# hrpan/tetris_mcts

Hardware: NVIDIA H100
Metric: mcts_sims_per_sec (higher is better)
Workload: dtype f32

## Files before the change

tetris_mcts_b200/_lib.py:

```python
import ctypes as C
import os

import numpy as np

HERE = os.path.dirname(os.path.abspath(__file__))
LIB_PATH = os.environ.get("B200_TETRIS_LIB") or os.path.join(HERE, "libb200_tetris_mcts.so")

REC_WORDS = 20
KEY_WORDS = 12
N_ACTIONS = 7
N_WEIGHTS = 478342

MODE_LP, MODE_SINGLE, MODE_VANILLA, MODE_DIST = 0, 1, 2, 3
EVAL_SYNTHETIC, EVAL_NET, EVAL_NET_TC = 0, 1, 2
ERR_NAMES = {1: "BAD_ARG", 2: "CUDA", 3: "ARENA_FULL", 4: "TRACE_FULL", 5: "NO_WEIGHTS"}


class B200Error(RuntimeError):
    def __init__(self, code, msg):
        super().__init__("b200 error %d (%s): %s" % (code, ERR_NAMES.get(code, "?"), msg))
        self.code = code


class Config(C.Structure):
# ... 13 lines not shown
    if _lib is None:
        if not os.path.exists(LIB_PATH):
            raise ImportError("%s is missing: run `python -m tetris_mcts_b200.build` (nvcc, sm_90a). "
                              "tetris_mcts_b200 has no CPU fallback." % LIB_PATH)
        L = C.CDLL(LIB_PATH)
        L.b200_last_error.restype = C.c_char_p
        L.b200_engine_create.argtypes = [C.POINTER(Config), C.POINTER(P)]
        L.b200_engine_destroy.argtypes = [P]
        L.b200_engine_set_stream.argtypes = [P, P]
        L.b200_engine_get_stream.argtypes = [P, C.POINTER(P)]
        L.b200_load_weights.argtypes = [P, P]
        L.b200_set_games.argtypes = [P, P]
        L.b200_get_games.argtypes = [P, P]
        L.b200_update_root.argtypes = [P, C.c_int]
        L.b200_run_sims.argtypes = [P, C.c_int]
        L.b200_get_stats.argtypes = [P, P, P]
        L.b200_env_step.argtypes = [P, P]
        L.b200_play_move.argtypes = [P, C.c_int, C.c_int, P, P]
        L.b200_status.argtypes = [P, P]
        L.b200_finished_games.argtypes = [P, P, C.c_int, P]
        L.b200_remove_nodes.argtypes = [P, C.c_int]
        L.b200_set_gc_headroom.argtypes = [P, C.c_int]
        L.b200_set_deep_lane.argtypes = [P, C.c_int]
        L.b200_set_path_cache.argtypes = [P, C.c_int]
        L.b200_counters.argtypes = [P, P]
        L.b200_sync.argtypes = [P]
        L.b200_set_timing.argtypes = [P, C.c_int]
        L.b200_timer_start.argtypes = [P]
        L.b200_timer_stop.argtypes = [P, P]
        L.b200_phase_ms.argtypes = [P, P, P]
        L.b200_export_game.argtypes = [P, C.c_int] + [P] * 13
        L.b200_valuenet_forward.argtypes = [P, P, C.c_int, P, P]
        L.b200_debug_act3.argtypes = [P, P, C.c_int, P]
        L.b200_tetris_step.argtypes = [P, P, C.c_int]
        L.b200_tetris_new.argtypes = [P, C.c_int, C.c_int, C.c_int, C.c_int, P, C.c_int]
        L.b200_tetris_state.argtypes = [P, P, C.c_int]
        L.b200_select_trace_obs.argtypes = [C.c_int] + [P] * 6 + [C.c_int, C.c_int, P, P, C.c_int, P]
        L.b200_backup_trace_obs.argtypes = [P, C.c_int] + [P] * 5 + [C.c_int, C.c_double, C.c_double, C.c_double]
        L.b200_backup_trace_obs_LP.argtypes = ([P, C.c_int] + [P] * 6 + [C.c_int, P, P, C.c_int, P, P, C.c_double,
                                               C.c_int, C.c_int])
        L.b200_get_unique_child_obs.argtypes = [C.c_int, P, P, P, C.c_int, P, P, P]
        L.b200_get_all_childs.argtypes = [C.c_int, P, C.c_int, P]
        L.b200_collect_samples_dev.argtypes = [P, C.c_int, P, C.c_int, P]
        L.b200_replay_enable.argtypes = [P, C.c_int, C.c_int]
        L.b200_replay_drain_dev.argtypes = [P, P, C.c_int, P]
        L.b200_replay_policy.argtypes = [P, C.c_int, C.c_int, C.c_int]
        L.b200_replay_policy_step.argtypes = [P, C.c_int64, P, P]
        L.b200_replay_policy_trained.argtypes = [P, C.c_int64]
        L.b200_replay_peek_dev.argtypes = [P, P, C.c_int]
        L.b200_replay_append.argtypes = [P, P, C.c_int]
        L.b200_load_dist_weights.argtypes = [P, P, C.c_int]
        L.b200_distnet_forward.argtypes = [P, P, C.c_int, C.c_int, P]
        L.b200_export_dist.argtypes = [P, C.c_int, P, P]
        L.b200_dist_shift_distribution.argtypes = [P, C.c_int, C.c_double, C.c_double, C.c_double, P]
        L.b200_dist_mean_variance.argtypes = [P, C.c_int, C.c_double, C.c_double, P, P]
        L.b200_dist_select_trace.argtypes = [C.c_int, P, P, C.c_int, C.c_int, P, P, C.c_int, P]
        L.b200_dist_backup_trace.argtypes = [P, C.c_int, P, P, C.c_int, C.c_int, C.c_double, P, C.c_double, C.c_double]
        _lib = L
    return _lib


def check(rc):
    if rc != 0:
        raise B200Error(rc, lib().b200_last_error().decode())


# ... 10 lines not shown
```

tetris_mcts_b200/csrc/capi.cu:

```cuda
#include <cuda_runtime.h>
#include <cmath>
#include <cstdio>
#include <cstdlib>
#include <cstring>
#include <string>
#include <vector>

#include "../../include/b200_tetris_mcts.h"
#include "kernels.cuh"
#include "valuenet_simt.cuh"
#include "dist_dev.cuh"
#include "distnet_simt.cuh"
#include "replay_policy.cuh"
#ifdef B200_WITH_TC
#include "valuenet_tc.cuh"
#include "distnet_tc.cuh"
#endif

using namespace b200;

static thread_local std::string g_err;
static int fail(int code, const std::string &msg) { g_err = msg; return code; }
#define CK(call)                                                                                      \
    do {                                                                                              \
// ... 18 lines not shown
    std::vector<void *> allocs;
    uint32_t *d_default_rec = nullptr;
    float *d_stats = nullptr; int32_t *d_action = nullptr;
    unsigned long long *d_game_stats = nullptr;
    bool have_weights = false;
    float *d_wraw = nullptr;
    NetWeights W{};
    float *d_act3 = nullptr; size_t act3_rows = 0;
    void *tc_state = nullptr; void *dn_tc_state = nullptr;
    bool have_dist_weights = false; float *d_dnw = nullptr; DistNetWeights DW{}; float *d_dn_act = nullptr; size_t dn_rows = 0;
    int n_sm = 132;
    bool timing = false;
    std::vector<cudaEvent_t> ev; size_t ev_used = 0;
    std::vector<int> ev_phase;
    float phase_ms[PH_N] = {0}; uint64_t phase_launches[PH_N] = {0};
    cudaEvent_t t0 = nullptr, t1 = nullptr;
    uint8_t *d_samples = nullptr; int sample_cap = 0; int32_t *d_sample_count = nullptr;
    ReplayPolicy rp; uint8_t *d_rp_tmp = nullptr, *d_rp_keep = nullptr; float *d_rp_vis = nullptr; int32_t *d_rp_kept = nullptr; int replay_alloc = 0;
    int gc_headroom = 0;
    int4 *d_pc = nullptr; int32_t *d_pc_var = nullptr, *d_pc_len = nullptr; uint4 *d_pc_sib = nullptr; int4 *d_pc_own = nullptr;
    int deep_cap = 0; cudaStream_t stream1 = nullptr; cudaEvent_t ev_fork = nullptr, ev_join = nullptr;
    int32_t *d_glist0 = nullptr, *d_glist1 = nullptr, *d_nlist = nullptr, *d_nreq_deep = nullptr, *d_gc_list_deep = nullptr; uint2 *d_req_deep = nullptr;
    int gc_pool_main = 0;
    cudaGraphExec_t step_exec = nullptr; bool step_graph_failed = false;
    uint64_t step_launches[PH_N] = {0};
};

static void drop_step_graph(b200_engine *e) {
    if (e->step_exec) { cudaStreamSynchronize(e->stream); cudaGraphExecDestroy(e->step_exec); e->step_exec = nullptr; }
    e->step_graph_failed = false;
}

constexpr int DEEP_GC_BLOCKS = 8;

static inline int backup_bitmap_words(const Arena &A) { return A.pc ? (A.M + 31) / 32 : 0; }
static inline size_t backup_smem(const Arena &A) { return (size_t)4 * backup_bitmap_words(A) * sizeof(unsigned); }

struct Scratch {
    std::vector<void *> bufs;
    ~Scratch() { for (void *q : bufs) cudaFree(q); }
    template <typename T> cudaError_t get(T **out, size_t bytes) {
        void *q = nullptr;
        cudaError_t err = cudaMalloc(&q, bytes ? bytes : 1);
        if (err == cudaSuccess) { bufs.push_back(q); *out = (T *)q; }
        return err;
    }
};

static void dfree(b200_engine *e, void *p) {
    if (!p) return;
    for (size_t i = 0; i < e->allocs.size(); ++i)
        if (e->allocs[i] == p) { e->allocs.erase(e->allocs.begin() + i); break; }
    cudaFree(p);
}

template <typename T>
static int dalloc(b200_engine *e, T **p, size_t n, bool zero = true) {
    void *q = nullptr;
    cudaError_t err = cudaMalloc(&q, n * sizeof(T));
    if (err != cudaSuccess) return fail(B200_ERR_CUDA, std::string("cudaMalloc ") + std::to_string(n * sizeof(T)) + " B: " + cudaGetErrorString(err));
    if (zero) cudaMemsetAsync(q, 0, n * sizeof(T), e->stream);
    e->allocs.push_back(q);
    *p = (T *)q;
    return 0;
}

// ... 67 lines not shown
    cudaDeviceProp prop;
    CK(cudaGetDeviceProperties(&prop, cfg->device));
    e->n_sm = prop.multiProcessorCount;
    Arena &A = e->A;
    memset(&A, 0, sizeof(A));
    A.G = cfg->n_games; A.M = cfg->max_nodes;
    int H = A.M + A.M / 2;
    if (H < 16) H = 16;
    A.H = H; A.trace_max = cfg->trace_max > 0 ? cfg->trace_max : 512;
    A.mode = cfg->mode; A.low = cfg->low; A.lp_end_from_obs = cfg->lp_end_from_obs; A.lp_var_gamma2 = cfg->lp_var_gamma2;
    A.stale_pop = cfg->stale_pop; A.eval_kind = cfg->eval_kind; A.overflow_reset = cfg->overflow_reset; A.gc_min_gain = cfg->overflow_reset ? cfg->max_nodes / 8 : 0; A.gamma = cfg->gamma; A.rollout_variance = cfg->rollout_variance;
    size_t GM = (size_t)A.G * A.M, G = (size_t)A.G;
    int rc = 0;
    rc |= dalloc(e, &A.row, GM * ROW_WORDS);
    rc |= dalloc(e, &A.stat, GM);
    rc |= dalloc(e, &A.rec, GM * REC_WORDS, false);
    rc |= dalloc(e, &A.key, GM * KEY_WORDS);
    rc |= dalloc(e, &A.ntab, G * H);
    rc |= dalloc(e, &A.otab, G * H);
    rc |= dalloc(e, &A.nfree, GM); rc |= dalloc(e, &A.ofree, GM);
    rc |= dalloc(e, &A.n_nfree, G); rc |= dalloc(e, &A.n_ofree, G);
    rc |= dalloc(e, &A.root, G); rc |= dalloc(e, &A.episode, G); rc |= dalloc(e, &A.status, G); rc |= dalloc(e, &A.srng, G);
    rc |= dalloc(e, &A.trace, G * A.trace_max); rc |= dalloc(e, &A.trace_len, G); rc |= dalloc(e, &A.leaf_kind, G);
    rc |= dalloc(e, &A.trace_meta, G * A.trace_max);
    {
        e->gc_pool_main = e->n_sm * 4 < A.G ? e->n_sm * 4 : A.G;
        const size_t pool = (size_t)(e->gc_pool_main + DEEP_GC_BLOCKS) * A.M;
        rc |= dalloc(e, &A.nmark, pool); rc |= dalloc(e, &A.omark, pool); rc |= dalloc(e, &A.gc_queue, pool * 2);
    }
    rc |= dalloc(e, &A.cur, G * REC_WORDS);
    rc |= dalloc(e, &A.req, G * 8); rc |= dalloc(e, &A.n_req, 4);
    rc |= dalloc(e, &A.gc_list, G); rc |= dalloc(e, &A.pending, G); rc |= dalloc(e, &A.resume_a, G);
    rc |= dalloc(e, &A.eval_out, G * 8); rc |= dalloc(e, &A.rollout_val, G);
    rc |= dalloc(e, &A.counters, 48);
    A.fin_cap = 4 * A.G;
    rc |= dalloc(e, &A.fin_log, (size_t)A.fin_cap * 4); rc |= dalloc(e, &A.fin_count, 1);
    if (cfg->mode == MODE_DIST) {
        A.dist_bins = cfg->dist_bins; A.dist_vmin = cfg->dist_vmin; A.dist_vmax = cfg->dist_vmax;
        rc |= dalloc(e, &A.nstat, GM * NSTAT_WORDS); rc |= dalloc(e, &A.ndist, GM * (size_t)A.dist_bins); rc |= dalloc(e, &A.dist_eval, G * (size_t)A.dist_bins);
    }
    rc |= dalloc(e, &e->d_default_rec, REC_WORDS);
    rc |= dalloc(e, &e->d_stats, G * 21); rc |= dalloc(e, &e->d_action, G);
    e->d_game_stats = A.counters + 8;
    float *zt = nullptr;
    rc |= dalloc(e, &zt, ZTABLE_N);
    if (rc) return B200_ERR_CUDA;
    {
        std::vector<float> h(ZTABLE_N);
        const double l2 = log(2.0), l22 = log(22.0), l41 = log(41.0);
        for (int n = 0; n < ZTABLE_N; ++n) {
            double t = (double)n, alpha = 1 - 1 / t;
            h[n] = (float)(10 * log(1 - log(-log(alpha) / l2) / l22) / l41);
        }
        CK(cudaMemcpyAsync(zt, h.data(), ZTABLE_N * sizeof(float), cudaMemcpyHostToDevice, e->stream));
        CK(cudaStreamSynchronize(e->stream));
        A.ztable = zt;
    }
    k_new_games<<<1, 1, 0, e->stream>>>(e->d_default_rec, 1, cfg->actions_per_drop, cfg->scoring, cfg->randomizer, nullptr, 0);
    k_init_arena<<<e->n_sm * 8, 256, 0, e->stream>>>(A, e->d_default_rec, cfg->seed);
    CK(cudaGetLastError());
    CK(cudaStreamSynchronize(e->stream));
    guard.e = nullptr;
    *out = e;
    return B200_OK;
}

extern "C" int b200_engine_destroy(b200_engine *e) {
// ... 73 lines not shown
    e->W.wfc1 = e->W.b1 + 96; e->W.bfc1 = e->W.wfc1 + (size_t)1792 * 256; e->W.wout = e->W.bfc1 + 256;
    e->W.bout = e->W.wout + 512; e->W.ub = e->W.bout + 2; e->W.lb = e->W.bout + 4;
    CK(cudaFuncSetAttribute(k_vn_conv, cudaFuncAttributeMaxDynamicSharedMemorySize, VN_SMEM_BYTES));
#ifdef B200_WITH_TC
    {
        int rc = tc_prepare(&e->tc_state, w, e->stream);
        if (rc) return fail(B200_ERR_CUDA, "tensor-core weight preparation failed");
    }
#endif
    e->have_weights = true;
    drop_step_graph(e);
    return B200_OK;
}

static int ensure_act3(b200_engine *e, size_t rows) {
    if (e->act3_rows >= rows) return 0;
    if (e->d_act3) { cudaStreamSynchronize(e->stream); dfree(e, e->d_act3); e->d_act3 = nullptr; e->act3_rows = 0; }
    if (dalloc(e, &e->d_act3, rows * 1792, false)) return B200_ERR_CUDA;
    e->act3_rows = rows;
    return 0;
}

static int launch_net(b200_engine *e, const uint2 *req, const int32_t *n_req, const uint32_t *keys, int M, float2 *eval_out,
                      size_t max_rows) {
    if (!e->have_weights) return fail(B200_ERR_NO_WEIGHTS, "b200_load_weights was not called");
#ifdef B200_WITH_TC
    if (e->cfg.eval_kind == B200_EVAL_NET_TC) {
        TcState *st = (TcState *)e->tc_state;
        const uint8_t *act3_before = st->d_act3;
        if (tc_ensure_act3(st, max_rows, e->stream)) return fail(B200_ERR_CUDA, "act3 (tensor-core layout) allocation failed");
        if (act3_before && st->d_act3 != act3_before) drop_step_graph(e);
        {
            PhaseTimer t(e, PH_CONV);
            k_tc_conv<<<e->n_sm, TCC_THREADS, TCC_SMEM, e->stream>>>(e->W, st->TW, req, n_req, nullptr, keys, M, st->d_act3, (int)st->tiles,
                                                                    e->timing ? e->A.counters + 16 : nullptr);
        }
        {
            PhaseTimer t(e, PH_FC);
            k_tc_fc<<<e->n_sm, TCF_THREADS, TCF_SMEM, e->stream>>>(e->W, st->TW, st->d_act3, (int)st->tiles, req, n_req, eval_out);
        }
        CK(cudaGetLastError());
        return B200_OK;
    }
#endif
    {
        const float *act3_before = e->d_act3;
        if (ensure_act3(e, max_rows)) return B200_ERR_CUDA;
        if (act3_before && e->d_act3 != act3_before) drop_step_graph(e);
    }
    {
        PhaseTimer t(e, PH_CONV);
        k_vn_conv<<<e->n_sm, VN_THREADS, VN_SMEM_BYTES, e->stream>>>(e->W, req, n_req, keys, M, e->d_act3);
    }
    {
        PhaseTimer t(e, PH_FC);
        k_vn_fc<<<e->n_sm * 2, FC_THREADS, 0, e->stream>>>(e->W, e->d_act3, req, n_req, eval_out);
    }
    CK(cudaGetLastError());
    return B200_OK;
}

__global__ void k_states_to_keys(const int8_t *states, int k, uint32_t *keys, uint2 *req);

extern "C" int b200_load_dist_weights(b200_engine *e, const float *w, int atoms) {
    if (!e || !w || atoms < 2 || atoms > 64) return fail(B200_ERR_BAD_ARG, "bad argument");
    CK(cudaSetDevice(e->cfg.device));
    if (e->A.mode == MODE_DIST && atoms != e->A.dist_bins) return fail(B200_ERR_BAD_ARG, "atoms must equal dist_bins");
    std::vector<float> h;
// ... 206 lines not shown
static int enqueue_step_lanes(b200_engine *e) {
    const Arena &A = e->A;
    const int G = A.G;
    if (!e->have_weights) return fail(B200_ERR_NO_WEIGHTS, "b200_load_weights was not called");
    TcState *st = (TcState *)e->tc_state;
    const uint8_t *act3_before = st->d_act3;
    if (tc_ensure_act3(st, (size_t)G * (A.mode == MODE_LP ? 7 : 1), e->stream)) return fail(B200_ERR_CUDA, "act3 (tensor-core layout) allocation failed");
    if (act3_before && st->d_act3 != act3_before) drop_step_graph(e);
    cudaStream_t s0 = e->stream, s1 = e->timing ? e->stream : e->stream1;
    Arena A0 = A, A1 = A;
    A0.glist = e->d_glist0; A0.n_list = e->d_nlist;
    A1.glist = e->d_glist1; A1.n_list = e->d_nlist + 1;
    A1.req = e->d_req_deep; A1.n_req = e->d_nreq_deep; A1.gc_list = e->d_gc_list_deep;
    A1.nmark += (size_t)e->gc_pool_main * A.M; A1.omark += (size_t)e->gc_pool_main * A.M; A1.gc_queue += (size_t)e->gc_pool_main * A.M * 2;
    A0.prof = e->timing ? A.counters + 32 : nullptr;
    CK(cudaMemsetAsync(A.n_req, 0, 4 * sizeof(int32_t), s0));
    CK(cudaMemsetAsync(e->d_nreq_deep, 0, 2 * sizeof(int32_t), s0));
    if (s1 != s0) { CK(cudaEventRecord(e->ev_fork, s0)); CK(cudaStreamWaitEvent(s1, e->ev_fork, 0)); }
    const int deep_groups = blocks_groups(e->deep_cap);
    {
        PhaseTimer t(e, PH_SELECT);
        k_select_expand<<<(G + SE_GAMES_PER_BLOCK - 1) / SE_GAMES_PER_BLOCK, TPB, 0, s0>>>(A0);
        k_select_expand<<<(e->deep_cap + SE_GAMES_PER_BLOCK - 1) / SE_GAMES_PER_BLOCK, TPB, 0, s1>>>(A1);
    }
    {
        PhaseTimer t(e, PH_GC);
        k_gc<<<gc_blocks(e), GC_THREADS, 0, s0>>>(A0);
        k_expand_resume<<<blocks_groups(G), TPB, 0, s0>>>(A0);
        k_gc<<<DEEP_GC_BLOCKS, GC_THREADS, 0, s1>>>(A1);
        k_expand_resume<<<deep_groups, TPB, 0, s1>>>(A1);
    }
    {
        PhaseTimer t(e, PH_CONV);
        k_tc_conv<<<e->n_sm, TCC_THREADS, TCC_SMEM, s0>>>(e->W, st->TW, A.req, A.n_req, nullptr, A.key, A.M, st->d_act3, (int)st->tiles,
                                                          e->timing ? A.counters + 16 : nullptr);
    }
    if (s1 != s0) { CK(cudaEventRecord(e->ev_join, s1)); CK(cudaStreamWaitEvent(s0, e->ev_join, 0)); }
    {
        PhaseTimer t(e, PH_CONV);
        k_merge_requests<<<1, 256, 0, s0>>>(A.req, A.n_req, e->d_req_deep, e->d_nreq_deep);
        k_tc_conv<<<e->n_sm, TCC_THREADS, TCC_SMEM, s0>>>(e->W, st->TW, A.req, A.n_req, A.n_req + 2, A.key, A.M, st->d_act3, (int)st->tiles, nullptr);
    }
    {
        PhaseTimer t(e, PH_FC);
        k_tc_fc<<<e->n_sm, TCF_THREADS, TCF_SMEM, s0>>>(e->W, st->TW, st->d_act3, (int)st->tiles, A.req, A.n_req, A.eval_out);
    }
    {
        PhaseTimer t(e, PH_BACKUP);
        k_backup<<<(G + 3) / 4, 128, backup_smem(A), s0>>>(A, backup_bitmap_words(A));
    }
    CK(cudaGetLastError());
    return B200_OK;
}
#endif

static int enqueue_step(b200_engine *e) {
    const Arena &A = e->A;
    const int G = A.G;
#ifdef B200_WITH_TC
    if (deep_lane_on(e)) return enqueue_step_lanes(e);
#endif
    CK(cudaMemsetAsync(A.n_req, 0, 2 * sizeof(int32_t), e->stream));
    {
        PhaseTimer t(e, PH_SELECT);
        Arena Ap = A;
        Ap.prof = e->timing ? A.counters + 32 : nullptr;
        k_select_expand<<<(G + SE_GAMES_PER_BLOCK - 1) / SE_GAMES_PER_BLOCK, TPB, 0, e->stream>>>(Ap);
    }
    {
        PhaseTimer t(e, PH_GC);
        k_gc<<<gc_blocks(e), GC_THREADS, 0, e->stream>>>(A);
        k_expand_resume<<<blocks_groups(G), TPB, 0, e->stream>>>(A);
    }
    if (A.mode == MODE_VANILLA) {
// ... 107 lines not shown
extern "C" int b200_finished_games(b200_engine *e, int32_t *out4, int cap, int32_t *count_out) {
    if (!e || !out4 || cap < 0 || !count_out) return fail(B200_ERR_BAD_ARG, "bad argument");
    CK(cudaSetDevice(e->cfg.device));
    int32_t n = 0;
    CK(cudaMemcpyAsync(&n, e->A.fin_count, 4, cudaMemcpyDeviceToHost, e->stream));
    CK(cudaStreamSynchronize(e->stream));
    *count_out = n;
    int m = n < e->A.fin_cap ? n : e->A.fin_cap;
    if (m > cap) m = cap;
    if (m > 0) CK(cudaMemcpyAsync(out4, e->A.fin_log, (size_t)m * 16, cudaMemcpyDeviceToHost, e->stream));
    CK(cudaMemsetAsync(e->A.fin_count, 0, 4, e->stream));
    CK(cudaStreamSynchronize(e->stream));
    return B200_OK;
}

extern "C" int b200_status(b200_engine *e, int32_t *status) {
    if (!e || !status) return fail(B200_ERR_BAD_ARG, "null argument");
    CK(cudaSetDevice(e->cfg.device));
    CK(cudaMemcpyAsync(status, e->A.status, (size_t)e->A.G * 4, cudaMemcpyDeviceToHost, e->stream));
    CK(cudaStreamSynchronize(e->stream));
    for (int g = 0; g < e->A.G; ++g)
        status[g] = (status[g] == ST_OK || status[g] == ST_RESET_DONE) ? 0 : (status[g] == ST_ARENA_FULL ? B200_ERR_ARENA_FULL : B200_ERR_TRACE_FULL);
    return B200_OK;
}

extern "C" int b200_counters(b200_engine *e, uint64_t *out16) {
    if (!e || !out16) return fail(B200_ERR_BAD_ARG, "null argument");
    CK(cudaSetDevice(e->cfg.device));
    CK(cudaMemcpyAsync(out16, e->A.counters, 16 * 8, cudaMemcpyDeviceToHost, e->stream));
    CK(cudaStreamSynchronize(e->stream));
    return B200_OK;
}

extern "C" int b200_debug_prof(b200_engine *e, uint64_t *out16) {
    if (!e || !out16) return fail(B200_ERR_BAD_ARG, "null argument");
    CK(cudaSetDevice(e->cfg.device));
    CK(cudaMemcpyAsync(out16, e->A.counters + 16, 16 * 8, cudaMemcpyDeviceToHost, e->stream));
    CK(cudaStreamSynchronize(e->stream));
    return B200_OK;
}

extern "C" int b200_debug_prof_tree(b200_engine *e, uint64_t *out16) {
    if (!e || !out16) return fail(B200_ERR_BAD_ARG, "null argument");
    CK(cudaSetDevice(e->cfg.device));
    CK(cudaMemcpyAsync(out16, e->A.counters + 32, 16 * 8, cudaMemcpyDeviceToHost, e->stream));
    CK(cudaStreamSynchronize(e->stream));
    return B200_OK;
}

extern "C" int b200_debug_trace_lens(b200_engine *e, int32_t *out) {
    if (!e || !out) return fail(B200_ERR_BAD_ARG, "null argument");
    CK(cudaSetDevice(e->cfg.device));
    CK(cudaMemcpyAsync(out, e->A.trace_len, (size_t)e->A.G * 4, cudaMemcpyDeviceToHost, e->stream));
    CK(cudaStreamSynchronize(e->stream));
    return B200_OK;
}

extern "C" int b200_sync(b200_engine *e) {
    if (!e) return fail(B200_ERR_BAD_ARG, "null engine");
    CK(cudaSetDevice(e->cfg.device));
    CK(cudaStreamSynchronize(e->stream));
    return B200_OK;
}

extern "C" int b200_timer_start(b200_engine *e) {
    if (!e) return fail(B200_ERR_BAD_ARG, "null engine");
    CK(cudaSetDevice(e->cfg.device));
    if (!e->t0) { CK(cudaEventCreate(&e->t0)); CK(cudaEventCreate(&e->t1)); }
    CK(cudaStreamSynchronize(e->stream));
    CK(cudaEventRecord(e->t0, e->stream));
// ... 606 lines not shown
```

tetris_mcts_b200/csrc/valuenet_tc.cuh:

```cuda
#pragma once
#include <cuda_fp16.h>
#include "search_dev.cuh"
#include "valuenet_simt.cuh"

namespace b200 {

__device__ __forceinline__ uint32_t smem_u32(const void *p) { return (uint32_t)__cvta_generic_to_shared(p); }

__device__ __forceinline__ void mbar_init(uint64_t *bar, uint32_t count) {
    asm volatile("mbarrier.init.shared::cta.b64 [%0], %1;" ::"r"(smem_u32(bar)), "r"(count));
}
__device__ __forceinline__ void mbar_wait(uint64_t *bar, uint32_t parity) {
    asm volatile(
        "{\n"
        ".reg .pred P1;\n"
        "LAB_WAIT:\n"
        "mbarrier.try_wait.parity.shared::cta.b64 P1, [%0], %1;\n"
        "@P1 bra DONE;\n"
        "bra LAB_WAIT;\n"
        "DONE:\n"
        "}" ::"r"(smem_u32(bar)), "r"(parity) : "memory");
}
__device__ __forceinline__ void mbar_arrive(uint64_t *bar) {
    asm volatile("mbarrier.arrive.shared::cta.b64 _, [%0];" ::"r"(smem_u32(bar)) : "memory");
// ... 96 lines not shown
          "+f"(d[72]), "+f"(d[73]), "+f"(d[74]), "+f"(d[75]), "+f"(d[76]), "+f"(d[77]), "+f"(d[78]), "+f"(d[79]),
          "+f"(d[80]), "+f"(d[81]), "+f"(d[82]), "+f"(d[83]), "+f"(d[84]), "+f"(d[85]), "+f"(d[86]), "+f"(d[87]),
          "+f"(d[88]), "+f"(d[89]), "+f"(d[90]), "+f"(d[91]), "+f"(d[92]), "+f"(d[93]), "+f"(d[94]), "+f"(d[95]),
          "+f"(d[96]), "+f"(d[97]), "+f"(d[98]), "+f"(d[99]), "+f"(d[100]), "+f"(d[101]), "+f"(d[102]), "+f"(d[103]),
          "+f"(d[104]), "+f"(d[105]), "+f"(d[106]), "+f"(d[107]), "+f"(d[108]), "+f"(d[109]), "+f"(d[110]), "+f"(d[111]),
          "+f"(d[112]), "+f"(d[113]), "+f"(d[114]), "+f"(d[115]), "+f"(d[116]), "+f"(d[117]), "+f"(d[118]), "+f"(d[119]),
          "+f"(d[120]), "+f"(d[121]), "+f"(d[122]), "+f"(d[123]), "+f"(d[124]), "+f"(d[125]), "+f"(d[126]), "+f"(d[127])
        : "l"(adesc), "l"(bdesc), "r"(accumulate));
}
__device__ __forceinline__ void split2(float x0, float x1, uint32_t &hi, uint32_t &lo) {
    const __half2 h = __floats2half2_rn(x0, x1);
    const float2 f = __half22float2(h);
    const __half2 l = __floats2half2_rn(x0 - f.x, x1 - f.y);
    hi = *reinterpret_cast<const uint32_t *>(&h); lo = *reinterpret_cast<const uint32_t *>(&l);
}

constexpr int TCC_WGS = 4;
constexpr int TCC_THREADS = TCC_WGS * 128;
constexpr int TCC_R = 144;
constexpr int TCC_WBLOCK = 2 * 2 * 96 * 16;
constexpr int TCC_WBYTES = 6 * TCC_WBLOCK;
constexpr int TCC_W1BYTES = 2 * 64 * 16;
constexpr int TCC_RUN = 4;
constexpr int TCC_ASLOT = 2 * 4 * TCC_R * 16;
constexpr int TCC_IMROWS = 192;
constexpr int TCC_IMSLOT = 2 * TCC_IMROWS * 16;
constexpr int TCC_OFF_W2 = 0;
constexpr int TCC_OFF_W3 = TCC_OFF_W2 + TCC_WBYTES;
constexpr int TCC_OFF_W1 = TCC_OFF_W3 + TCC_WBYTES;
constexpr int TCC_OFF_A1 = TCC_OFF_W1 + TCC_W1BYTES;
constexpr int TCC_OFF_IM = TCC_OFF_A1 + TCC_WGS * TCC_ASLOT;
constexpr int TCC_OFF_BIAS = TCC_OFF_IM + TCC_WGS * TCC_IMSLOT;
constexpr int TCC_OFF_KEY = TCC_OFF_BIAS + 96 * 4;
constexpr int TCC_SMEM = TCC_OFF_KEY + TCC_WGS * 32 * 4;
constexpr int ACT3_KCHUNKS = 224;
static_assert(TCC_SMEM <= 227 * 1024, "k_tc_conv shared memory");

struct TcWeights {
    const uint8_t *wc1;
    const uint8_t *wc2, *wc3;
    const uint8_t *wfc;
};

__device__ __forceinline__ size_t act3_off(int split, int n_tiles, int ridx, int kchunk) {
    return ((((size_t)split * n_tiles + (ridx >> 7)) * ACT3_KCHUNKS + kchunk) * 128 + (ridx & 127)) * 16;
}

__device__ __forceinline__ void issue_conv_layer(float (&d)[48], uint32_t a_addr, uint32_t w_addr) {
    const uint64_t a0 = gmma_desc(a_addr, TCC_R * 16, 128), b0 = gmma_desc(w_addr, 96 * 16, 128);
#pragma unroll
    for (int dy = 0; dy < 3; ++dy) {
#pragma unroll
        for (int h = 0; h < 2; ++h) {
            const uint32_t a_hi = 2 * h * TCC_R + dy * 8, a_lo = a_hi + 4 * TCC_R;
            const uint32_t b_hi = (dy * 2 + h) * (TCC_WBLOCK / 16), b_lo = b_hi + 2 * 96;
            wgmma_n96(d, a0 + a_hi, b0 + b_hi, (dy | h) ? 1u : 0u);
            wgmma_n96(d, a0 + a_hi, b0 + b_lo, 1u);
            wgmma_n96(d, a0 + a_lo, b0 + b_hi, 1u);
        }
    }
}

__device__ __forceinline__ void build_im2col3(uint8_t *im, const uint32_t *tab, int wt) {
    for (int p = wt; p < TCC_R; p += 128) {
        const int y = p >> 3, x = p & 7;
        uint32_t hv[9];
#pragma unroll
        for (int dy = 0; dy < 3; ++dy) {
            const uint32_t rw = tab[y + dy] >> x;
#pragma unroll
            for (int dx = 0; dx < 3; ++dx)
                hv[dy * 3 + dx] = ((rw >> dx) & 1u) * 0x3C00u | ((rw >> (16 + dx)) & 1u) * 0xBC00u;
        }
        *reinterpret_cast<uint4 *>(im + p * 16) =
            make_uint4(hv[0] | (hv[1] << 16), hv[2] | (hv[3] << 16), hv[4] | (hv[5] << 16), hv[6] | (hv[7] << 16));
        *reinterpret_cast<uint32_t *>(im + TCC_IMROWS * 16 + p * 16) = hv[8];
    }
}

__global__ void __launch_bounds__(TCC_THREADS, 1)
k_tc_conv(NetWeights W, TcWeights TW, const uint2 *req, const int32_t *n_req_ptr, const int32_t *first_ptr, const uint32_t *keys, int M, uint8_t *act3,
          int n_tiles, unsigned long long *prof) {
    extern __shared__ __align__(128) uint8_t smem[];
    float *sB = reinterpret_cast<float *>(smem + TCC_OFF_BIAS);
    const int t = threadIdx.x, wg = t >> 7, wt = t & 127, w = wt >> 5, lane = t & 31;
    for (int i = t; i < TCC_WBYTES / 16; i += TCC_THREADS) {
        reinterpret_cast<uint4 *>(smem + TCC_OFF_W2)[i] = reinterpret_cast<const uint4 *>(TW.wc2)[i];
        reinterpret_cast<uint4 *>(smem + TCC_OFF_W3)[i] = reinterpret_cast<const uint4 *>(TW.wc3)[i];
    }
    for (int i = t; i < TCC_W1BYTES / 16; i += TCC_THREADS) reinterpret_cast<uint4 *>(smem + TCC_OFF_W1)[i] = reinterpret_cast<const uint4 *>(TW.wc1)[i];
    for (int i = t; i < (TCC_OFF_BIAS - TCC_OFF_A1) / 16; i += TCC_THREADS) reinterpret_cast<uint4 *>(smem + TCC_OFF_A1)[i] = make_uint4(0, 0, 0, 0);
    if (t < 32) { sB[t] = W.b1[t] * TC_SCALE_A; sB[32 + t] = W.b2[t] * TC_SCALE_A; sB[64 + t] = W.b3[t] * TC_SCALE_A; }
    fence_async_smem();
    __syncthreads();
    const int first = first_ptr ? *first_ptr : 0;
    const int n_req = *n_req_ptr - first;
    const int n_workers = (int)gridDim.x * TCC_WGS, wid = (int)blockIdx.x * TCC_WGS + wg;
    const int n_runs = (n_req + TCC_RUN - 1) / TCC_RUN;
    int n_local = 0;
    for (int run = wid; run < n_runs; run += n_workers) n_local += min(TCC_RUN, n_req - run * TCC_RUN);
    auto board_of = [&](int i) -> int { return first + ((i / TCC_RUN) * n_workers + wid) * TCC_RUN + (i % TCC_RUN); };
    uint8_t *act = smem + TCC_OFF_A1 + wg * TCC_ASLOT, *im = smem + TCC_OFF_IM + wg * TCC_IMSLOT;
    uint32_t *sKey = reinterpret_cast<uint32_t *>(smem + TCC_OFF_KEY) + wg * 32;
    const uint32_t s_act = smem_u32(act), s_im = smem_u32(im);
    const uint32_t s_w1 = smem_u32(smem + TCC_OFF_W1), s_w2 = smem_u32(smem + TCC_OFF_W2), s_w3 = smem_u32(smem + TCC_OFF_W3);
    const int qd = lane & 3, rl = lane >> 2;
    constexpr float K23 = TC_UNSCALE * TC_SCALE_A, K1 = TC_SCALE_A / TC_SCALE_W;
    constexpr int SPLIT = 4 * TCC_R * 16;
    const bool do_prof = prof && blockIdx.x == 0 && t == 0;
    long long pacc[4] = {0, 0, 0, 0}, ptick = clock64();
    auto prof_t = [&](int k) { if (do_prof) { const long long n = clock64(); pacc[k] += n - ptick; ptick = n; } };
    auto fetch = [&](int i) -> uint32_t {
        if (i >= n_local || lane >= 12) return 0u;
        const uint2 rq = req[board_of(i)];
        return keys[((size_t)rq.x * M + (rq.y & 0x0fffffffu)) * KEY_WORDS + lane];
    };
    uint32_t kw = w == 0 ? fetch(0) : 0u;
    for (int i = 0; i < n_local; ++i) {
        const int ridx = board_of(i);
        if (w == 0) {
            const uint32_t rowpair = __shfl_sync(0xffffffffu, kw, (lane >> 1) & 15), pcs = __shfl_sync(0xffffffffu, kw, 10);
            uint32_t tab = (rowpair >> ((lane & 1) * 16)) & 0x3ffu;
#pragma unroll
            for (int k = 0; k < 4; ++k) {
                const uint32_t cell = (pcs >> (8 * k)) & 0xffu, pr = (cell * 205u) >> 11, pcol = cell - pr * 10u;
                tab |= (pr == (uint32_t)lane ? 1u : 0u) << (16 + pcol);
            }
            kw = fetch(i + 1);
            if (lane < 20) sKey[lane] = tab;
        }
        wg_sync(wg);
        build_im2col3(im, sKey, wt);
        fence_async_smem();
        wg_sync(wg);
        prof_t(0);
#pragma unroll 1
        for (int mt = 0; mt < 3; ++mt) {
            float d[32];
#pragma unroll
            for (int k = 0; k < 32; ++k) d[k] = 0.f;
            wgmma_fence();
            wgmma_n64(d, gmma_desc(s_im + mt * 1024, TCC_IMROWS * 16, 128), gmma_desc(s_w1, 64 * 16, 128), 0u);
            wgmma_commit();
            wgmma_wait<0>();
            fence_regs(d);
#pragma unroll
            for (int h = 0; h < 2; ++h) {
                const int r = mt * 64 + 16 * w + 8 * h + rl;
                if (r < TCC_R) {
#pragma unroll
                    for (int j = 0; j < 4; ++j) {
                        const int c = 8 * j + 2 * qd;
                        const float o0 = fmaxf(fmaf(d[4 * (j + 4) + 2 * h] + d[4 * j + 2 * h], K1, sB[c]), 0.f);
                        const float o1 = fmaxf(fmaf(d[4 * (j + 4) + 2 * h + 1] + d[4 * j + 2 * h + 1], K1, sB[c + 1]), 0.f);
                        uint32_t hi, lo;
                        split2(o0, o1, hi, lo);
                        uint8_t *dst = act + (j * TCC_R + r) * 16 + qd * 4;
                        *reinterpret_cast<uint32_t *>(dst) = hi;
                        *reinterpret_cast<uint32_t *>(dst + SPLIT) = lo;
                    }
                }
            }
        }
        fence_async_smem();
        wg_sync(wg);
        prof_t(1);
#pragma unroll 1
        for (int layer = 0; layer < 2; ++layer) {
            const float *bias = sB + 32 * (layer + 1);
#pragma unroll 1
            for (int mt = 0; mt < 2; ++mt) {
                float d[48];
#pragma unroll
                for (int k = 0; k < 48; ++k) d[k] = 0.f;
                wgmma_fence();
                issue_conv_layer(d, s_act + mt * 1024, layer ? s_w3 : s_w2);
                wgmma_commit();
                wgmma_wait<0>();
                fence_regs(d);
#pragma unroll
                for (int h = 0; h < 2; ++h) {
                    const int y = mt * 8 + 2 * w + h, x = rl;
#pragma unroll
                    for (int j = 0; j < 4; ++j) {
                        float o[2];
#pragma unroll
                        for (int e = 0; e < 2; ++e) {
                            const int k = 4 * j + 2 * h + e;
                            const float s1 = __shfl_down_sync(0xffffffffu, d[16 + k], 4), s2 = __shfl_down_sync(0xffffffffu, d[32 + k], 8);
                            o[e] = fmaxf(fmaf((s2 + s1) + d[k], K23, bias[8 * j + 2 * qd + e]), 0.f);
                        }
                        uint32_t hi, lo;
                        split2(o[0], o[1], hi, lo);
                        if (layer == 0) {
                            if (x < 6) {
                                uint8_t *dst = act + (j * TCC_R + y * 8 + x) * 16 + qd * 4;
                                *reinterpret_cast<uint32_t *>(dst) = hi;
                                *reinterpret_cast<uint32_t *>(dst + SPLIT) = lo;
                            }
                        } else if (y < 14 && x < 4) {
                            const int kc = (y * 4 + x) * 4 + j;
                            *reinterpret_cast<uint32_t *>(act3 + act3_off(0, n_tiles, ridx, kc) + qd * 4) = hi;
                            *reinterpret_cast<uint32_t *>(act3 + act3_off(1, n_tiles, ridx, kc) + qd * 4) = lo;
                        }
                    }
                }
            }
            fence_async_smem();
            wg_sync(wg);
            prof_t(2 + layer);
        }
    }
    if (do_prof) for (int k = 0; k < 4; ++k) atomicAdd(&prof[k], (unsigned long long)pacc[k]);
}

constexpr int TCF_CONSUMERS = 2;
constexpr int TCF_PRODUCER = TCF_CONSUMERS * 4;
constexpr int TCF_THREADS = TCF_CONSUMERS * 128 + 32;
constexpr int TCF_STAGES = 8;
constexpr int TCF_A_BYTES = 2 * 128 * 16;
constexpr int TCF_B_BYTES = 2 * 256 * 16;
constexpr int TCF_STAGE = 2 * TCF_A_BYTES + 2 * TCF_B_BYTES;
constexpr int TCF_KBLOCKS = 112;
constexpr int TCF_OFF_BAR = TCF_STAGES * TCF_STAGE;
constexpr int TCF_OFF_EPI = TCF_OFF_BAR + 256;
static_assert(2 * TCF_STAGES * 8 <= 256, "barrier block overflows into the epilogue constants");
constexpr int TCF_SMEM = TCF_OFF_EPI + (256 * 3 + 8) * 4;
static_assert(TCF_SMEM <= 227 * 1024, "k_tc_fc shared memory");

__global__ void __launch_bounds__(TCF_THREADS, 1)
k_tc_fc(NetWeights W, TcWeights TW, const uint8_t *act3, int n_tiles_alloc, const uint2 *req, const int32_t *n_req_ptr, float2 *eval_out) {
    extern __shared__ __align__(128) uint8_t smem[];
    uint64_t *full = reinterpret_cast<uint64_t *>(smem + TCF_OFF_BAR);
    uint64_t *empty = full + TCF_STAGES;
    float *sBias = reinterpret_cast<float *>(smem + TCF_OFF_EPI), *sWo = sBias + 256, *sTail = sWo + 512;
    const int t = threadIdx.x, warp = t >> 5, lane = t & 31;
    for (int i = t; i < 256; i += TCF_THREADS) { sBias[i] = W.bfc1[i]; sWo[i] = W.wout[i]; sWo[256 + i] = W.wout[256 + i]; }
    if (t < 2) { sTail[t] = W.bout[t]; sTail[2 + t] = W.ub[t]; sTail[4 + t] = W.lb[t]; }
    if (t == 0) {
        for (int i = 0; i < TCF_STAGES; ++i) { mbar_init(&full[i], 1); mbar_init(&empty[i], TCF_CONSUMERS); }
        fence_barrier_init();
    }
    __syncthreads();
    const int n_req = *n_req_ptr;
    const int n_tiles = (n_req + 127) >> 7;
    if (warp == TCF_PRODUCER) {
// ... 98 lines not shown
                uint16_t s2[2] = {0, 0};
                if (tap < 9) host_split2(c1w[n * 9 + tap] * TC_SCALE_W, s2);
                for (int s = 0; s < 2; ++s) p1[((size_t)c2 * 64 + s * 32 + n) * 8 + e] = s2[s];
            }
    for (int layer = 0; layer < 2; ++layer) {
        const float *cw = layer ? c3w : c2w;
        uint16_t *dst = layer ? p3 : p2;
        for (int dy = 0; dy < 3; ++dy)
            for (int hh = 0; hh < 2; ++hh)
                for (int c2 = 0; c2 < 2; ++c2)
                    for (int dx = 0; dx < 3; ++dx)
                        for (int n = 0; n < 32; ++n)
                            for (int e = 0; e < 8; ++e) {
                                int ci = 16 * hh + 8 * c2 + e;
                                uint16_t s2[2];
                                host_split2(cw[(n * 32 + ci) * 9 + dy * 3 + dx] * TC_SCALE_W, s2);
                                for (int s = 0; s < 2; ++s)
                                    dst[(((((size_t)(dy * 2 + hh)) * 2 + s) * 2 + c2) * 96 + dx * 32 + n) * 8 + e] = s2[s];
                            }
    }
    for (int j = 0; j < TCF_KBLOCKS; ++j)
        for (int c2 = 0; c2 < 2; ++c2)
            for (int n = 0; n < 256; ++n)
                for (int e = 0; e < 8; ++e) {
                    int kp = j * 16 + c2 * 8 + e, p = kp >> 5, c = kp & 31;
                    uint16_t s2[2];
                    host_split2(f1w[(size_t)n * 1792 + c * 56 + p] * TC_SCALE_W, s2);
                    for (int s = 0; s < 2; ++s) pf[((((size_t)s * TCF_KBLOCKS + j) * 2 + c2) * 256 + n) * 8 + e] = s2[s];
                }
    if (!st->d_w && cudaMalloc(&st->d_w, h.size()) != cudaSuccess) return 1;
    if (cudaMemcpyAsync(st->d_w, h.data(), h.size(), cudaMemcpyHostToDevice, stream) != cudaSuccess) return 1;
    if (cudaStreamSynchronize(stream) != cudaSuccess) return 1;
    st->TW.wc1 = st->d_w; st->TW.wc2 = st->d_w + TCC_W1BYTES; st->TW.wc3 = st->TW.wc2 + TCC_WBYTES; st->TW.wfc = st->TW.wc3 + TCC_WBYTES;
    if (cudaFuncSetAttribute(k_tc_conv, cudaFuncAttributeMaxDynamicSharedMemorySize, TCC_SMEM) != cudaSuccess) return 1;
    if (cudaFuncSetAttribute(k_tc_fc, cudaFuncAttributeMaxDynamicSharedMemorySize, TCF_SMEM) != cudaSuccess) return 1;
    return 0;
}

static int tc_ensure_act3(TcState *st, size_t max_rows, cudaStream_t stream) {
    size_t tiles = (max_rows + 127) / 128;
    if (st->tiles >= tiles) return 0;
    if (st->d_act3) { cudaStreamSynchronize(stream); cudaFree(st->d_act3); st->d_act3 = nullptr; }
    size_t bytes = (size_t)2 * tiles * ACT3_KCHUNKS * 2048;
    if (cudaMalloc(&st->d_act3, bytes) != cudaSuccess) return 1;
    cudaMemsetAsync(st->d_act3, 0, bytes, stream);
    st->tiles = tiles;
    return 0;
}

static void tc_destroy(void *state) {
    TcState *st = (TcState *)state;
    if (!st) return;
    cudaFree(st->d_w); cudaFree(st->d_act3);
    delete st;
}

}
```

tetris_mcts_b200/engine.py:

```python
import ctypes as C
import os

import numpy as np

from . import _lib as L


PATH_CACHE_DEFAULT = "1"


class BatchedEngine:
    def __init__(self, n_games, max_nodes=8192, mode="lp", gamma=None, low=None, eval_kind="net", weights=None,
                 env_args=((20, 10), 1, 0, 0), seed=123, device=0, lp_end_from_obs=False, lp_var_gamma2=True,
                 stale_pop=True, rollout_variance=1e3, trace_max=512, overflow_reset=False, dist_bins=50, dist_vmin=0.0, dist_vmax=5000.0,
                 dist_weights=None, path_cache=None):
        mode_id = {"lp": L.MODE_LP, "single": L.MODE_SINGLE, "vanilla": L.MODE_VANILLA, "dist": L.MODE_DIST}[mode] if isinstance(mode, str) else int(mode)
        eval_id = {"synthetic": L.EVAL_SYNTHETIC, "net": L.EVAL_NET, "net_tc": L.EVAL_NET_TC}[eval_kind] if isinstance(eval_kind, str) else int(eval_kind)
        if tuple(env_args[0]) != (20, 10):
            raise ValueError("only 20x10 boards (SPEC_PYTETRIS.md §1)")
        cfg = L.Config()
        cfg.n_games, cfg.max_nodes, cfg.mode = int(n_games), int(max_nodes), mode_id
        cfg.gamma = float(gamma if gamma is not None else (0.99 if mode_id == L.MODE_VANILLA else 0.999))
        cfg.low = int(low if low is not None else (5 if mode_id in (L.MODE_VANILLA, L.MODE_DIST) else 1))
        cfg.dist_bins, cfg.dist_vmin, cfg.dist_vmax = int(dist_bins), float(dist_vmin), float(dist_vmax)
# ... 120 lines not shown

    def status(self):
        st = np.zeros(self.n_games, np.int32)
        L.check(L.lib().b200_status(self.h, L.ptr(st)))
        return st

    COUNTER_NAMES = ("sims", "expansions", "eval_requests", "gcs", "trace_levels", "rollout_steps", "new_nodes", "tree_resets",
                     "games_finished", "score_sum", "lines_sum", "_11", "max_trace_len", "cached_levels")

    def counters(self):
        c = np.zeros(16, np.uint64)
        L.check(L.lib().b200_counters(self.h, L.ptr(c)))
        return {n: int(c[i]) for i, n in enumerate(self.COUNTER_NAMES) if not n.startswith("_")}

    PHASES = ("select_expand", "conv", "fc", "backup", "rollout", "synthetic", "misc", "gc")

    def timer_start(self):
        L.check(L.lib().b200_timer_start(self.h))

    def timer_stop(self):
        ms = np.zeros(1, np.float32)
        L.check(L.lib().b200_timer_stop(self.h, L.ptr(ms)))
        return float(ms[0])

    def set_timing(self, on=True):
        L.check(L.lib().b200_set_timing(self.h, int(on)))

    def phase_ms(self):
        ms = np.zeros(8, np.float32)
        n = np.zeros(8, np.uint64)
        L.check(L.lib().b200_phase_ms(self.h, L.ptr(ms), L.ptr(n)))
        return {p: (float(ms[i]), int(n[i])) for i, p in enumerate(self.PHASES) if not p.startswith("_")}

    def export_game(self, game):
        M = self.max_nodes
        d = dict(child=np.zeros((M, 7), np.int32), score=np.zeros(M, np.float32), episode=np.zeros(M, np.int32),
                 n2o=np.zeros(M, np.int32), visit=np.zeros(M, np.int32), value=np.zeros(M, np.float32),
                 variance=np.zeros(M, np.float32), obs_end=np.zeros(M, np.uint8),
                 game=np.zeros((M, L.REC_WORDS), np.uint32), obs_key=np.zeros((M, L.KEY_WORDS), np.uint32))
        root = np.zeros(1, np.int32)
        tr = np.zeros(int(self.cfg.trace_max) or 512, np.int32)
        tl = np.zeros(1, np.int32)
        L.check(L.lib().b200_export_game(self.h, int(game), L.ptr(d["child"]), L.ptr(d["score"]), L.ptr(d["episode"]),
                                         L.ptr(d["n2o"]), L.ptr(d["visit"]), L.ptr(d["value"]), L.ptr(d["variance"]),
                                         L.ptr(d["obs_end"]), L.ptr(d["game"]), L.ptr(d["obs_key"]), L.ptr(root),
                                         L.ptr(tr), L.ptr(tl)))
        d["root"] = int(root[0])
        d["last_trace"] = tr[:int(tl[0])].copy()
        return d

    def valuenet(self, states):
        s = np.ascontiguousarray(states, np.int8).reshape(-1, 200)
        v = np.zeros(len(s), np.float32)
        var = np.zeros(len(s), np.float32)
        L.check(L.lib().b200_valuenet_forward(self.h, L.ptr(s), len(s), L.ptr(v), L.ptr(var)))
        return v, var

    def replay_enable(self, min_visits=25, capacity=500000):
        L.check(L.lib().b200_replay_enable(self.h, int(min_visits), int(capacity)))

    def replay_drain_into(self, dev_ptr, capacity):
        cnt = np.zeros(1, np.int32)
        L.check(L.lib().b200_replay_drain_dev(self.h, C.c_void_p(int(dev_ptr)), int(capacity), L.ptr(cnt)))
        return int(cnt[0])

    def replay_policy(self, accumulation_policy, episodes_per_train=25, memory_growth_rate=5000):
# ... 22 lines not shown
```

Baseline: 8.491 million.

## Pipeline conv1 wgmma tiles, drop trailing sync, template out conv profiling

```diff
diff --git a/tetris_mcts_b200/_lib.py b/tetris_mcts_b200/_lib.py
--- a/tetris_mcts_b200/_lib.py
+++ b/tetris_mcts_b200/_lib.py
@@ -69,6 +69,7 @@
         L.b200_export_game.argtypes = [P, C.c_int] + [P] * 13
         L.b200_valuenet_forward.argtypes = [P, P, C.c_int, P, P]
         L.b200_debug_act3.argtypes = [P, P, C.c_int, P]
+        L.b200_debug_prof.argtypes = [P, P]
         L.b200_tetris_step.argtypes = [P, P, C.c_int]
         L.b200_tetris_new.argtypes = [P, C.c_int, C.c_int, C.c_int, C.c_int, P, C.c_int]
         L.b200_tetris_state.argtypes = [P, P, C.c_int]
diff --git a/tetris_mcts_b200/csrc/capi.cu b/tetris_mcts_b200/csrc/capi.cu
--- a/tetris_mcts_b200/csrc/capi.cu
+++ b/tetris_mcts_b200/csrc/capi.cu
@@ -74,6 +74,10 @@
 }
 
 constexpr int DEEP_GC_BLOCKS = 8;
+constexpr int CONV_PROF_AT = 48, CONV_PROF_WORDS = 24;
+#ifdef B200_WITH_TC
+static_assert(TCC_WGS * TCC_PROF_WORDS == CONV_PROF_WORDS, "k_tc_conv probe words");
+#endif
 
 static inline int backup_bitmap_words(const Arena &A) { return A.pc ? (A.M + 31) / 32 : 0; }
 static inline size_t backup_smem(const Arena &A) { return (size_t)4 * backup_bitmap_words(A) * sizeof(unsigned); }
@@ -207,7 +211,7 @@
     rc |= dalloc(e, &A.req, G * 8); rc |= dalloc(e, &A.n_req, 4);
     rc |= dalloc(e, &A.gc_list, G); rc |= dalloc(e, &A.pending, G); rc |= dalloc(e, &A.resume_a, G);
     rc |= dalloc(e, &A.eval_out, G * 8); rc |= dalloc(e, &A.rollout_val, G);
-    rc |= dalloc(e, &A.counters, 48);
+    rc |= dalloc(e, &A.counters, CONV_PROF_AT + CONV_PROF_WORDS);
     A.fin_cap = 4 * A.G;
     rc |= dalloc(e, &A.fin_log, (size_t)A.fin_cap * 4); rc |= dalloc(e, &A.fin_count, 1);
     if (cfg->mode == MODE_DIST) {
@@ -347,8 +351,11 @@
         if (act3_before && st->d_act3 != act3_before) drop_step_graph(e);
         {
             PhaseTimer t(e, PH_CONV);
-            k_tc_conv<<<e->n_sm, TCC_THREADS, TCC_SMEM, e->stream>>>(e->W, st->TW, req, n_req, nullptr, keys, M, st->d_act3, (int)st->tiles,
-                                                                    e->timing ? e->A.counters + 16 : nullptr);
+            if (e->timing)
+                k_tc_conv<true><<<e->n_sm, TCC_THREADS, TCC_SMEM, e->stream>>>(e->W, st->TW, req, n_req, nullptr, keys, M, st->d_act3, (int)st->tiles,
+                                                                              e->A.counters + CONV_PROF_AT);
+            else
+                k_tc_conv<false><<<e->n_sm, TCC_THREADS, TCC_SMEM, e->stream>>>(e->W, st->TW, req, n_req, nullptr, keys, M, st->d_act3, (int)st->tiles, nullptr);
         }
         {
             PhaseTimer t(e, PH_FC);
@@ -621,14 +628,17 @@
     }
     {
         PhaseTimer t(e, PH_CONV);
-        k_tc_conv<<<e->n_sm, TCC_THREADS, TCC_SMEM, s0>>>(e->W, st->TW, A.req, A.n_req, nullptr, A.key, A.M, st->d_act3, (int)st->tiles,
-                                                          e->timing ? A.counters + 16 : nullptr);
+        if (e->timing)
+            k_tc_conv<true><<<e->n_sm, TCC_THREADS, TCC_SMEM, s0>>>(e->W, st->TW, A.req, A.n_req, nullptr, A.key, A.M, st->d_act3, (int)st->tiles,
+                                                                    A.counters + CONV_PROF_AT);
+        else
+            k_tc_conv<false><<<e->n_sm, TCC_THREADS, TCC_SMEM, s0>>>(e->W, st->TW, A.req, A.n_req, nullptr, A.key, A.M, st->d_act3, (int)st->tiles, nullptr);
     }
     if (s1 != s0) { CK(cudaEventRecord(e->ev_join, s1)); CK(cudaStreamWaitEvent(s0, e->ev_join, 0)); }
     {
         PhaseTimer t(e, PH_CONV);
         k_merge_requests<<<1, 256, 0, s0>>>(A.req, A.n_req, e->d_req_deep, e->d_nreq_deep);
-        k_tc_conv<<<e->n_sm, TCC_THREADS, TCC_SMEM, s0>>>(e->W, st->TW, A.req, A.n_req, A.n_req + 2, A.key, A.M, st->d_act3, (int)st->tiles, nullptr);
+        k_tc_conv<false><<<e->n_sm, TCC_THREADS, TCC_SMEM, s0>>>(e->W, st->TW, A.req, A.n_req, A.n_req + 2, A.key, A.M, st->d_act3, (int)st->tiles, nullptr);
     }
     {
         PhaseTimer t(e, PH_FC);
@@ -802,10 +812,10 @@
     return B200_OK;
 }
 
-extern "C" int b200_debug_prof(b200_engine *e, uint64_t *out16) {
-    if (!e || !out16) return fail(B200_ERR_BAD_ARG, "null argument");
-    CK(cudaSetDevice(e->cfg.device));
-    CK(cudaMemcpyAsync(out16, e->A.counters + 16, 16 * 8, cudaMemcpyDeviceToHost, e->stream));
+extern "C" int b200_debug_prof(b200_engine *e, uint64_t *out24) {
+    if (!e || !out24) return fail(B200_ERR_BAD_ARG, "null argument");
+    CK(cudaSetDevice(e->cfg.device));
+    CK(cudaMemcpyAsync(out24, e->A.counters + CONV_PROF_AT, CONV_PROF_WORDS * 8, cudaMemcpyDeviceToHost, e->stream));
     CK(cudaStreamSynchronize(e->stream));
     return B200_OK;
 }
diff --git a/tetris_mcts_b200/csrc/valuenet_tc.cuh b/tetris_mcts_b200/csrc/valuenet_tc.cuh
--- a/tetris_mcts_b200/csrc/valuenet_tc.cuh
+++ b/tetris_mcts_b200/csrc/valuenet_tc.cuh
@@ -152,7 +152,8 @@
 constexpr int TCC_OFF_IM = TCC_OFF_A1 + TCC_WGS * TCC_ASLOT;
 constexpr int TCC_OFF_BIAS = TCC_OFF_IM + TCC_WGS * TCC_IMSLOT;
 constexpr int TCC_OFF_KEY = TCC_OFF_BIAS + 96 * 4;
-constexpr int TCC_SMEM = TCC_OFF_KEY + TCC_WGS * 32 * 4;
+constexpr int TCC_OFF_PROF = TCC_OFF_KEY + TCC_WGS * 32 * 4;
+constexpr int TCC_SMEM = TCC_OFF_PROF + TCC_WGS * 8 * 4;
 constexpr int ACT3_KCHUNKS = 224;
 static_assert(TCC_SMEM <= 227 * 1024, "k_tc_conv shared memory");
 
@@ -198,6 +199,19 @@
     }
 }
 
+constexpr int TCC_PROF_EVERY = 8;
+enum TcProf {
+    TCP_BOARDS,
+    TCP_MMA,
+    TCP_EPI,
+    TCP_SYNC,
+    TCP_CONV1,
+    TCP_OTHER,
+    TCC_PROF_WORDS
+};
+static_assert(TCC_PROF_WORDS <= 8, "probe words per warpgroup in shared memory");
+
+template <bool PROF>
 __global__ void __launch_bounds__(TCC_THREADS, 1)
 k_tc_conv(NetWeights W, TcWeights TW, const uint2 *req, const int32_t *n_req_ptr, const int32_t *first_ptr, const uint32_t *keys, int M, uint8_t *act3,
           int n_tiles, unsigned long long *prof) {
@@ -227,9 +241,12 @@
     const int qd = lane & 3, rl = lane >> 2;
     constexpr float K23 = TC_UNSCALE * TC_SCALE_A, K1 = TC_SCALE_A / TC_SCALE_W;
     constexpr int SPLIT = 4 * TCC_R * 16;
-    const bool do_prof = prof && blockIdx.x == 0 && t == 0;
-    long long pacc[4] = {0, 0, 0, 0}, ptick = clock64();
-    auto prof_t = [&](int k) { if (do_prof) { const long long n = clock64(); pacc[k] += n - ptick; ptick = n; } };
+    const bool do_prof = PROF && blockIdx.x % TCC_PROF_EVERY == 0 && wt == 0;
+    uint32_t *sProf = reinterpret_cast<uint32_t *>(smem + TCC_OFF_PROF) + wg * 8;
+    if (PROF && do_prof) for (int k = 0; k < TCC_PROF_WORDS; ++k) sProf[k] = 0u;
+    uint32_t ptick = PROF ? (uint32_t)clock() : 0u;
+    auto lap = [&](int bucket) { if (PROF && do_prof) { const uint32_t n = (uint32_t)clock(); sProf[bucket] += n - ptick; ptick = n; } };
+    auto sync_wg = [&]() { lap(TCP_OTHER); wg_sync(wg); lap(TCP_SYNC); };
     auto fetch = [&](int i) -> uint32_t {
         if (i >= n_local || lane >= 12) return 0u;
         const uint2 rq = req[board_of(i)];
@@ -249,20 +266,11 @@
             kw = fetch(i + 1);
             if (lane < 20) sKey[lane] = tab;
         }
-        wg_sync(wg);
+        sync_wg();
         build_im2col3(im, sKey, wt);
         fence_async_smem();
-        wg_sync(wg);
-        prof_t(0);
-#pragma unroll 1
-        for (int mt = 0; mt < 3; ++mt) {
-            float d[32];
-#pragma unroll
-            for (int k = 0; k < 32; ++k) d[k] = 0.f;
-            wgmma_fence();
-            wgmma_n64(d, gmma_desc(s_im + mt * 1024, TCC_IMROWS * 16, 128), gmma_desc(s_w1, 64 * 16, 128), 0u);
-            wgmma_commit();
-            wgmma_wait<0>();
+        sync_wg();
+        auto conv1_epilogue = [&](float (&d)[32], int mt) {
             fence_regs(d);
 #pragma unroll
             for (int h = 0; h < 2; ++h) {
@@ -281,10 +289,29 @@
                     }
                 }
             }
+        };
+        {
+            float d0[32], d1[32], d2[32];
+#pragma unroll
+            for (int k = 0; k < 32; ++k) { d0[k] = 0.f; d1[k] = 0.f; d2[k] = 0.f; }
+            const uint64_t b1 = gmma_desc(s_w1, 64 * 16, 128);
+            wgmma_fence();
+            wgmma_n64(d0, gmma_desc(s_im, TCC_IMROWS * 16, 128), b1, 0u);
+            wgmma_commit();
+            wgmma_n64(d1, gmma_desc(s_im + 1024, TCC_IMROWS * 16, 128), b1, 0u);
+            wgmma_commit();
+            wgmma_n64(d2, gmma_desc(s_im + 2048, TCC_IMROWS * 16, 128), b1, 0u);
+            wgmma_commit();
+            wgmma_wait<2>();
+            conv1_epilogue(d0, 0);
+            wgmma_wait<1>();
+            conv1_epilogue(d1, 1);
+            wgmma_wait<0>();
+            conv1_epilogue(d2, 2);
         }
         fence_async_smem();
-        wg_sync(wg);
-        prof_t(1);
+        lap(TCP_CONV1);
+        sync_wg();
 #pragma unroll 1
         for (int layer = 0; layer < 2; ++layer) {
             const float *bias = sB + 32 * (layer + 1);
@@ -293,11 +320,13 @@
                 float d[48];
 #pragma unroll
                 for (int k = 0; k < 48; ++k) d[k] = 0.f;
+                lap(TCP_OTHER);
                 wgmma_fence();
                 issue_conv_layer(d, s_act + mt * 1024, layer ? s_w3 : s_w2);
                 wgmma_commit();
                 wgmma_wait<0>();
                 fence_regs(d);
+                lap(TCP_MMA);
 #pragma unroll
                 for (int h = 0; h < 2; ++h) {
                     const int y = mt * 8 + 2 * w + h, x = rl;
@@ -325,13 +354,19 @@
                         }
                     }
                 }
-            }
-            fence_async_smem();
-            wg_sync(wg);
-            prof_t(2 + layer);
-        }
-    }
-    if (do_prof) for (int k = 0; k < 4; ++k) atomicAdd(&prof[k], (unsigned long long)pacc[k]);
+                lap(TCP_EPI);
+            }
+            if (layer == 0) {
+                fence_async_smem();
+                sync_wg();
+            }
+        }
+    }
+    if (PROF && do_prof) {
+        lap(TCP_OTHER);
+        sProf[TCP_BOARDS] = (uint32_t)n_local;
+        for (int k = 0; k < TCC_PROF_WORDS; ++k) atomicAdd(&prof[wg * TCC_PROF_WORDS + k], (unsigned long long)sProf[k]);
+    }
 }
 
 constexpr int TCF_CONSUMERS = 2;
@@ -496,7 +531,8 @@
     if (cudaMemcpyAsync(st->d_w, h.data(), h.size(), cudaMemcpyHostToDevice, stream) != cudaSuccess) return 1;
     if (cudaStreamSynchronize(stream) != cudaSuccess) return 1;
     st->TW.wc1 = st->d_w; st->TW.wc2 = st->d_w + TCC_W1BYTES; st->TW.wc3 = st->TW.wc2 + TCC_WBYTES; st->TW.wfc = st->TW.wc3 + TCC_WBYTES;
-    if (cudaFuncSetAttribute(k_tc_conv, cudaFuncAttributeMaxDynamicSharedMemorySize, TCC_SMEM) != cudaSuccess) return 1;
+    if (cudaFuncSetAttribute(k_tc_conv<false>, cudaFuncAttributeMaxDynamicSharedMemorySize, TCC_SMEM) != cudaSuccess) return 1;
+    if (cudaFuncSetAttribute(k_tc_conv<true>, cudaFuncAttributeMaxDynamicSharedMemorySize, TCC_SMEM) != cudaSuccess) return 1;
     if (cudaFuncSetAttribute(k_tc_fc, cudaFuncAttributeMaxDynamicSharedMemorySize, TCF_SMEM) != cudaSuccess) return 1;
     return 0;
 }
diff --git a/tetris_mcts_b200/engine.py b/tetris_mcts_b200/engine.py
--- a/tetris_mcts_b200/engine.py
+++ b/tetris_mcts_b200/engine.py
@@ -176,6 +176,14 @@
         L.check(L.lib().b200_phase_ms(self.h, L.ptr(ms), L.ptr(n)))
         return {p: (float(ms[i]), int(n[i])) for i, p in enumerate(self.PHASES) if not p.startswith("_")}
 
+    CONV_PROBE = ("boards", "mma", "epilogue", "wg_sync", "conv1", "other")
+
+    def conv_probe(self):
+        c = np.zeros(24, np.uint64)
+        L.check(L.lib().b200_debug_prof(self.h, L.ptr(c)))
+        n = len(self.CONV_PROBE)
+        return [{k: int(c[n * wg + i]) for i, k in enumerate(self.CONV_PROBE)} for wg in range(4)]
+
     def export_game(self, game):
         M = self.max_nodes
         d = dict(child=np.zeros((M, 7), np.int32), score=np.zeros(M, np.float32), episode=np.zeros(M, np.int32),
```

Result: no change. 8.552 million, median of 6 (+0.7%).
